# rasmusab/bayes.js

Hardware: AMD Instinct MI355X
Metric: posterior draws/sec (= param-updates/sec) (higher is better)
Workload: dtype f64

## Files before the change

### bayes.js_amd/csrc/amwg_kernel.h

```cpp
#pragma once
#if !defined(__HIPCC_RTC__)
#include <hip/hip_runtime.h>
#endif

#include "amwg_div.h"
#include "amwg_ld.h"
#include "amwg_philox.h"
#include "amwg_types.h"

namespace amwg {

struct LdsLayout {
  uint32_t data, state, pls, cnt, tot, cc, adapt, pl, idx, perm, total, stride, logpls, bc, xw;
};
__host__ __device__ inline LdsLayout lds_layout(size_t data_bytes, int P, int CPB, int max_top, int n_named, bool multi = false) {
  LdsLayout L;
  uint32_t o = 0;
  L.stride = (uint32_t)P | 1u;
  L.data = o;  o += (uint32_t)((data_bytes + 15) & ~(size_t)15);
  L.state = o; o += L.stride * CPB * 8;
  L.pls = o;   o += L.stride * CPB * 8;
  L.cnt = o;   o += L.stride * CPB * 8;
  L.tot = o;   o += (L.stride * CPB * 4 + 15) & ~15u;
  L.cc = o;    o += (uint32_t)P * sizeof(CompConst);
  L.adapt = o; o += ((uint32_t)P + 7) & ~7u;
  L.pl = o;    o += (uint32_t)n_named * 20u;
  o = (o + 15) & ~15u;
  L.idx = o;   o += (max_top > 1) ? (((uint32_t)max_top * CPB * (max_top > kByteTop ? 2u : 1u) + 15) & ~15u) : 0;
  L.perm = o;  o += (n_named > kPackedNamed) ? (((uint32_t)n_named * CPB * 2u + 15) & ~15u) : 0;
  L.logpls = o; o += multi ? L.stride * CPB * 8 : 0;
  L.bc = o;     o += multi ? ((L.stride * CPB * 4 + 15) & ~15u) : 0;
  L.xw = o;     o += multi ? 2u * 16u * 8u : 0;
  L.total = (o + 15) & ~15u;
  return L;
}

template <class Model, bool FAST, int G, int U = Model::kUnroll>
__device__ __forceinline__ double pass_over_data(const typename Model::Pass &ps, int n_obs, int sub, double acc) {
  const int n_full = n_obs / G, rem = n_obs % G;
  int k = 0;
  for (; k + U <= n_full; k += U) {
    double t[U];
#pragma unroll
    for (int u = 0; u < U; ++u) t[u] = Model::template term<FAST>(ps, (k + u) * G + sub);
#pragma unroll
    for (int u = 0; u < U; ++u) acc += t[u];
  }
  for (; k < n_full; ++k) acc += Model::template term<FAST>(ps, k * G + sub);
  if (sub < rem) acc += Model::template term<FAST>(ps, n_full * G + sub);
  return acc;
}

struct CrossWave {
  double *buf;
  int parity;
};

template <class...> using void_of = void;

template <class M, class = void> struct BinaryOf { static constexpr bool value = true; };
template <class M> struct BinaryOf<M, void_of<decltype(M::kHasBinary)>> { static constexpr bool value = M::kHasBinary; };

template <class M, class = void> struct TracksState { static constexpr bool value = false; };
template <class M> struct TracksState<M, void_of<decltype(M::kTracksState)>> { static constexpr bool value = M::kTracksState; };

// ... 170 lines not shown
  }
  __device__ __forceinline__ void set_block(const Philox4 &w) { u0 = u53(w.w0, w.w1); u1 = u53(w.w2, w.w3); }
  __device__ __forceinline__ void fill() { set_block(block(b0 + (uint64_t)lane_in_chain, c2, c3, k0, k1)); }
  __device__ __forceinline__ void init(uint64_t seed, uint64_t chain, uint64_t consumed, int tid) {
    k0 = (uint32_t)seed; k1 = (uint32_t)(seed >> 32);
    c2 = (uint32_t)chain; c3 = (uint32_t)(chain >> 32);
    lane_in_chain = tid & (L - 1);
    base_lane = (tid & 63) & ~(L - 1);
    b0 = consumed >> 1;
    pos = (uint32_t)(consumed & 1u);
    fill();
  }
  __device__ __forceinline__ uint64_t consumed() const { return 2 * b0 + (uint64_t)pos; }
  __device__ __forceinline__ double next() {
    if constexpr (L == 64) {
      uint32_t p = (uint32_t)__builtin_amdgcn_readfirstlane((int)pos);
      if (p >= 128u) { b0 += 64ull; p = 0u; fill(); }
      const double mine = (p & 1u) ? u1 : u0;
      const int src = (int)(p >> 1);
      const uint32_t hi = (uint32_t)__builtin_amdgcn_readlane((int)(f64_bits(mine) >> 32), src);
      const uint32_t lo = (uint32_t)__builtin_amdgcn_readlane((int)(uint32_t)f64_bits(mine), src);
      pos = p + 1u;
      return bits_f64(((uint64_t)hi << 32) | (uint64_t)lo);
    } else {
      if (pos >= 2u * (uint32_t)L) { b0 += (uint64_t)L; pos = 0u; fill(); }
      double mine = (pos & 1u) ? u1 : u0;
      if constexpr (L > 1) mine = __shfl(mine, base_lane + (int)(pos >> 1), 64);
      ++pos;
      return mine;
    }
  }
};

template <int G>
__device__ __forceinline__ bool chain_true(bool c) {
#if defined(__HIP_DEVICE_COMPILE__)
  if constexpr (G >= 64) return __ballot(c) != 0ull;
#endif
  return c;
}

__device__ inline __attribute__((noinline)) int certified_test_wide(double dA, double eta, double u) {
  const double lo = dA - eta, hi = dA + eta;
  if (hi < -746.0) return -1;
  if (lo >= 0.0) return 1;
  if (!(eta < 0x1p+9) || !(u > 0x1p-60)) return 0;
  if (exp_v8(lo) * (1.0 - 0x1p-50) > u) return 1;
  if (exp_v8(hi) * (1.0 + 0x1p-50) < u) return -1;
  return 0;
}
__device__ __forceinline__ int certified_test(double dA, double eta, double ex, double u) {
  if (eta < 0x1p-7) return (ex * (1.0 - eta) > u && (u > 0.0 || dA > -700.0)) ? 1 : (ex * (1.0 + eta) < u ? -1 : 0);
  return certified_test_wide(dA, eta, u);
}

template <class Rng>
__device__ __forceinline__ double rnorm_js(Rng &rng, double mean, double sd) {
  constexpr int GU = Rng::kLanesPerChain;
  double u, v, q;
  bool again;
  do {
    u = rng.next();
    v = 1.7156 * (rng.next() - 0.5);
    const double x = u - 0.449871;
    const double y = __builtin_fabs(v) + 0.386595;
    q = x * x + y * (0.19600 * y - 0.25472 * x);
    again = false;
    if (chain_true<GU>(q > 0.27597)) again = chain_true<GU>(q > 0.27846) || chain_true<GU>(v * v > -4 * log_v8_cold(u) * u * u);
  } while (again);
  return (v / u) * sd + mean;
}

struct IndexColumn {
  unsigned char *base;
  int CPB;
  bool wide;
  __device__ __forceinline__ int get(int t) const {
    return wide ? (int)reinterpret_cast<const uint16_t *>(base)[t * CPB] : (int)base[t * CPB];
  }
  __device__ __forceinline__ void set(int t, int v) const {
    if (wide) reinterpret_cast<uint16_t *>(base)[t * CPB] = (uint16_t)v; else base[t * CPB] = (uint8_t)v;
  }
};
__device__ __forceinline__ uint32_t perm_get(uint64_t perm, int i) { return (uint32_t)(perm >> (4 * i)) & 0xFu; }
__device__ __forceinline__ uint64_t perm_swap(uint64_t perm, int i, int j) {
  const uint64_t d = ((perm >> (4 * i)) ^ (perm >> (4 * j))) & 0xFull;
  return perm ^ (d << (4 * i)) ^ (d << (4 * j));
}

__device__ __forceinline__ double js_max2(double a, double b) {
  if (a != a || b != b) return __builtin_nan("");
  if (a == b) return (a == 0 && __builtin_signbit(a)) ? b : a;
  return a > b ? a : b;
}

template <class M, int G, bool GL, bool SW = false> struct RngOf { using type = CoopStream<G>; };
template <class M, int G> struct RngOf<M, G, true, false> { using type = typename M::Stream; };
template <class M, int G> struct RngOf<M, G, false, true> { using type = typename M::SweepStream; };
template <class M, class = void> struct DynamicLdsOf { static constexpr bool value = false; };
template <class M> struct DynamicLdsOf<M, void_of<decltype(M::kDynamicLds)>> { static constexpr bool value = M::kDynamicLds; };
template <class M, bool GL> struct DataBytesOf {
  static __device__ __forceinline__ size_t get(const DataRef &d, int lanes, int threads) {
    if constexpr (DynamicLdsOf<M>::value) return M::lds_bytes_of(d, lanes, threads);
    else return M::lds_bytes(d.n_obs, d.G, lanes);
  }
};
template <class M> struct DataBytesOf<M, true> { static __device__ __forceinline__ size_t get(const DataRef &d, int, int threads) { return M::gl_lds_bytes(d.pad, threads / 64); } };

#if defined(__HIP_DEVICE_COMPILE__)
typedef const StepArgs __attribute__((address_space(4))) *cold_args_ptr;
__device__ __forceinline__ cold_args_ptr cold_args() {
  cold_args_ptr p = (cold_args_ptr)__builtin_amdgcn_kernarg_segment_ptr();
  asm volatile("" : "+s"(p));
  return p;
}
#else
typedef const StepArgs *cold_args_ptr;
__device__ inline cold_args_ptr cold_args() { return nullptr; }
#endif

struct SlotPre {
  int comp;
  double cur, sd, batch_size;
  int2 cnt;
  bool adapting;
};

__device__ __forceinline__ uint64_t uniform_u64(uint64_t v) {
#if defined(__HIP_DEVICE_COMPILE__)
  return ((uint64_t)(uint32_t)__builtin_amdgcn_readfirstlane((int)(uint32_t)(v >> 32)) << 32) | (uint64_t)(uint32_t)__builtin_amdgcn_readfirstlane((int)(uint32_t)v);
// ... 68 lines not shown
}

__device__ __forceinline__ double lane_value(double v, int src) {
#if defined(__HIP_DEVICE_COMPILE__)
  const uint32_t hi = (uint32_t)__builtin_amdgcn_readlane((int)(f64_bits(v) >> 32), src);
  const uint32_t lo = (uint32_t)__builtin_amdgcn_readlane((int)(uint32_t)f64_bits(v), src);
  return bits_f64(((uint64_t)hi << 32) | (uint64_t)lo);
#else
  return v;
#endif
}

constexpr int kErrReplicasNeedOneWave = 1, kErrLaunchTooLong = 2, kErrMirrorOutOfSync = 4, kErrSweepNeedsOrderInRegisters = 8, kErrNoKernelBody = 16;
__device__ __forceinline__ void device_error(const StepArgs &a, int code) {
#if defined(__HIP_DEVICE_COMPILE__)
  if (threadIdx.x == 0) (void)atomicOr(a.ch.error, code);
#endif
}
template <class M, class = void> struct MirrorCheckOf { static constexpr bool value = false; };
template <class M> struct MirrorCheckOf<M, void_of<decltype(M::kMirrorCheck)>> { static constexpr bool value = M::kMirrorCheck; };

template <class Model, int G, int BT = 256, bool GL = false, bool SW = false, bool CT = false>
__device__ __forceinline__ void step_body(const StepArgs &a, unsigned char *smem) {
  constexpr int kPassU = SW ? (CertNeedsRows<Model>::value ? 2 : 4) : (BT >= 1024 ? 4 : 8);
  const int tid = threadIdx.x, nt = blockDim.x;
  constexpr bool kMulti = G > 64;
  if (!kMulti && a.cpb > 0 && nt != 64) { device_error(a, kErrReplicasNeedOneWave); return; }
  if (a.n_steps > 65535) { device_error(a, kErrLaunchTooLong); return; }
  const int CPB = kMulti ? G / 64 : ((a.cpb > 0 && a.cpb < nt / G) ? a.cpb : nt / G);
  const int c_raw = kMulti ? tid / 64 : tid / G;
  const int c_in = c_raw < CPB ? c_raw : CPB - 1, sub = tid % G;
  const int P = a.pl.P;
  const int n_named = a.pl.n_params;
  const LdsLayout L = lds_layout(DataBytesOf<Model, GL>::get(a.d, G, nt), P, CPB, a.pl.max_top, n_named, kMulti);

  const unsigned char *data_lds = smem + L.data;
  double *Sblk = reinterpret_cast<double *>(smem + L.state);
  CompConst *cc = reinterpret_cast<CompConst *>(smem + L.cc);
  uint8_t *adapt = smem + L.adapt;
  int32_t *pl_base = reinterpret_cast<int32_t *>(smem + L.pl), *pl_len = pl_base + n_named, *pl_top = pl_len + n_named, *pl_multidim = pl_top + n_named, *pl_inner = pl_multidim + n_named;
  const bool wide_idx = a.pl.max_top > kByteTop, wide_perm = n_named > kPackedNamed;
  const IndexColumn idx{smem + L.idx + (wide_idx ? 2 * c_in : c_in), CPB, wide_idx};
  const IndexColumn pcol{smem + L.perm + 2 * c_in, CPB, true};
  double *SDme = reinterpret_cast<double *>(smem + L.pls) + (size_t)c_in * L.stride;
  int2 *CNTme = reinterpret_cast<int2 *>(smem + L.cnt) + (size_t)c_in * L.stride;
  uint32_t *TOTme = reinterpret_cast<uint32_t *>(smem + L.tot) + (size_t)c_in * L.stride;
  double *LOGPLSme = reinterpret_cast<double *>(smem + L.logpls) + (size_t)c_in * L.stride;
  int32_t *BCme = reinterpret_cast<int32_t *>(smem + L.bc) + (size_t)c_in * L.stride;
  CrossWave xw{reinterpret_cast<double *>(smem + L.xw), 0};
  typename CacheOf<Model>::type cache = CacheOf<Model>::init();

  Model::stage(smem + L.data, a.d, tid, nt, G);
  for (int p = tid; p < P; p += nt) { cc[p] = a.cc[p]; adapt[p] = a.is_adapting[p]; }
  for (int i = tid; i < 4 * n_named; i += nt) pl_base[i] = a.pl.tab[i];
  for (int i = tid; i < n_named; i += nt) pl_inner[i] = a.pl.tab[n_named + i] / a.pl.tab[2 * n_named + i];

  const int64_t chain_raw = kMulti ? (int64_t)blockIdx.x : (int64_t)blockIdx.x * CPB + c_in;
  const bool live = chain_raw < a.C;
  const int64_t cl = live ? chain_raw : a.C - 1;
  const bool writer = live && sub == 0;
  const bool counter = sub == 0 && c_raw < CPB;
  const int64_t C = a.C;

  double *Sme = Sblk + (size_t)c_in * L.stride;
  for (int p = 0; p < P; ++p) {
    Sme[p] = a.ch.state[p * C + cl];
    SDme[p] = exp_v8(a.ch.prop_log_scale[p * C + cl]);
    CNTme[p] = make_int2(a.ch.acceptance_count[p * C + cl], a.ch.iterations_since_adaption[p * C + cl]);
    TOTme[p] = 0u;
    if constexpr (kMulti) { LOGPLSme[p] = a.ch.prop_log_scale[p * C + cl]; BCme[p] = a.ch.batch_count[p * C + cl]; }
  }
  const StateView S{Sme};
  uint64_t perm = wide_perm ? 0ull : a.ch.perm[cl];
  if (wide_perm)
    for (int k = 0; k < n_named; ++k) pcol.set(k, (int)a.ch.perm16[(int64_t)k * C + cl]);
  typename RngOf<Model, G, GL, SW>::type rng;
  if constexpr (GL) rng.init(a.seed, a.chain_offset + (uint64_t)cl, a.ch.rng_n[cl], tid, reinterpret_cast<double *>(smem + L.data + Model::gl_lds_bytes(a.d.pad, 0)) + (size_t)(tid >> 6) * 256);
  else if constexpr (SW) rng.init(a.seed, a.chain_offset + (uint64_t)cl, a.ch.rng_n[cl], tid, reinterpret_cast<double *>(smem + L.data + Model::window_offset(a.d, nt / 64)) + (size_t)(tid >> 6) * 256);
  else rng.init(a.seed, a.chain_offset + (uint64_t)cl, a.ch.rng_n[cl], tid);
  double lp_curr = a.ch.lp_curr[cl];
  __syncthreads();
  constexpr bool kCert = CT && CertifiedAt<Model, G>::value && !GL && (SW == CertNeedsRows<Model>::value);
  static_assert(kCert == CT, "a certified kernel is instantiated for a model that has no certified value at this lane count");
  constexpr bool kRefOrder = kCert && G > 1 && RefOrderOf<Model>::value;
  auto expression = [&]() -> double {
    if constexpr (kRefOrder) return Model::template reference_order<G>(cache, S, a.mc, a.d, data_lds, sub);
    else if constexpr (!GL) return log_post<Model, G, kPassU>(S, a, data_lds, sub, xw, cache);
    else return 0.0;
  };
  if constexpr (!GL) { if (a.init_lp) lp_curr = expression(); }
  double lpA = lp_curr, epsA = 0.0;
  bool lp_exact = true;
  if constexpr (kCert) { if (!a.init_lp) { epsA = a.ch.lp_eps[cl]; lp_exact = epsA == 0.0; } }
  (void)lpA; (void)epsA; (void)lp_exact;
#if defined(AMWG_AUDIT)
  constexpr bool kAudit = kCert;
#else
  constexpr bool kAudit = false;
#endif
  [[maybe_unused]] double audE = 0.0, aud_max_v = 0.0, aud_max_d = 0.0;
  [[maybe_unused]] uint32_t aud_n = 0u, aud_bad = 0u;
  [[maybe_unused]] auto audit_bin = [&](int which, double ratio) {
#if defined(AMWG_AUDIT)
    if (writer) {
      int b = 0;
      if (ratio > 0.0) { b = (int)((f64_bits(ratio) >> 52) & 0x7ffu) - 1023 + 40; b = b < 1 ? 1 : (b > 63 ? 63 : b); }
      if (!(ratio == ratio)) b = 63;
      (void)atomicAdd(cold_args()->ch.audit_hist + which * 64 + b, 1ull);
    }
#endif
  };
// ... 44 lines not shown

  const int lane64 = tid & 63;
  int ord = lane64;
  (void)ord;
  if (SW && a.pl.max_top > 64) { device_error(a, kErrSweepNeedsOrderInRegisters); return; }
  const bool ord_in_regs = SW ? true : (G >= 64 && a.pl.max_top <= 64);
  constexpr bool kSweep = SW && !GL && LaneReuseOf<Model>::value && G == 64 && !BinaryOf<Model>::value;
  const bool sweep_rt = kSweep && ord_in_regs && a.d.pad > 0;
  if constexpr (kAudit) { if (lp_exact) audE = lp_curr; else audE = expression(); }
  wave_priority(kStepperPriority);
  auto record_draws = [&](int step) {
    if (recording && step == next_rec) {
      double *const draws = cold_args()->draws;
      {
        constexpr int LW = G < 64 ? G : 64;
        if (live && (!kMulti || sub < 64))
          for (int p = sub & (LW - 1); p < P; p += LW) {
#if !defined(AMWG_X_NOREC)
            draws[(row * PR + p) * C + cl] = S(p);
#endif
          }
      }
      if constexpr (D > 0) {
        double dv[D];
        (void)Model::template eval<G, true>(S, a.d, data_lds, sub, dv);
        if (writer)
          for (int q = 0; q < D; ++q) draws[(row * PR + P + q) * C + cl] = dv[q];
      }
      ++row;
      next_rec += cold_args()->thin;
    }
  };
  auto shuffle_named = [&]() {
    for (int i = n_named - 1; i > 0; --i) {
      const int j = (int)__builtin_floor(rng.next() * (double)(i + 1));
      if (wide_perm) { const int ti = pcol.get(i); pcol.set(i, pcol.get(j)); pcol.set(j, ti); }
      else perm = perm_swap(perm, i, j);
    }
  };
  auto adapt_component = [&](int comp, bool accepted, int2 cnt, double batch_size, bool store, bool per_lane = false) {
    cnt.x += accepted ? 1 : 0;
    cnt.y += 1;
    const bool boundary = (double)cnt.y >= batch_size;
    if (per_lane ? boundary : chain_true<GL ? 1 : G>(boundary)) {
      const CompConst k = cc[comp];
      const int64_t gi = (int64_t)comp * C + cl;
      int32_t *const g_bc = kMulti ? nullptr : cold_args()->ch.batch_count;
      double *const g_pls = kMulti ? nullptr : cold_args()->ch.prop_log_scale;
      const int32_t bc = (kMulti ? BCme[comp] : g_bc[gi]) + 1;
      const double adj = __builtin_fmin(k.max_adaptation, k.initial_adaptation / __builtin_sqrt((double)bc));
      double pls = kMulti ? LOGPLSme[comp] : g_pls[gi];
      if ((double)cnt.x / k.batch_size > k.target_accept_rate) pls += adj; else pls -= adj;
      cnt = make_int2(0, 0);
      SDme[comp] = exp_v8_cold(pls);
      if constexpr (kMulti) { BCme[comp] = bc; LOGPLSme[comp] = pls; }
      else if (store) { g_bc[gi] = bc; g_pls[gi] = pls; }
    }
    CNTme[comp] = cnt;
  };

  [[maybe_unused]] auto accept_sweep = [&](double diff, double u_accept) -> bool {
    bool accepted = false;
    if (chain_true<G>(diff >= 0.0)) accepted = true;
    else if (chain_true<G>(diff < -746.0)) accepted = false;
    else {
      const double lower = 1.0 + diff;
// ... 532 lines not shown
        else {
          const double lower = 1.0 + diff;
          if (chain_true<G>(u_accept < lower - 0x1p-50)) accepted = true;
          else if (chain_true<G>(diff > -1.0 && u_accept > (lower + 0.5 * diff * diff) + 0x1p-50)) accepted = false;
          else accepted = chain_true<G>(exp_v8(diff) > u_accept);
        }
        accepted = chain_true<G>(accepted);
        if (accepted) lp_curr = prop_lp;
        else set_state(comp, cur);
        if constexpr (kCert) { lpA = lp_curr; epsA = 0.0; }
        if (counter) (void)__hip_atomic_fetch_add(&TOTme[comp], 1u + (accepted ? 0x10000u : 0u), __ATOMIC_RELAXED, __HIP_MEMORY_SCOPE_WORKGROUP);
      }
      if constexpr (kAudit) { if (inb && accepted) audE = aud_E_prop; }
      AMWG_PHASE(11);
      if (chain_true<G>(me.adapting)) adapt_component(comp, accepted, me.cnt, me.batch_size, writer);
      AMWG_PHASE(12);
    }
  }

  if constexpr (kCert) {
    if (a.finalize_lp && !lp_exact) { lp_curr = expression(); lp_exact = true; }
    if (!lp_exact) lp_curr = lpA;
    if (writer) cold_args()->ch.lp_eps[cl] = lp_exact ? 0.0 : epsA;
  }
  if constexpr (!GL && MirrorCheckOf<Model>::value) {
    if (!Model::template mirror_ok<G>(cache, S, a.d, sub)) (void)atomicOr(cold_args()->ch.error, kErrMirrorOutOfSync);
  }
#if defined(AMWG_X_PHASES)
  if ((tid & 63) == 0 && live) {
    unsigned long long *const hh = cold_args()->ch.audit_hist + 64;
#pragma unroll
    for (int q = 0; q < 16; ++q) (void)atomicAdd(hh + q, (unsigned long long)ph_acc[q]);
  }
#endif
  if constexpr (kAudit) {
    if (writer) {
      double *const au = cold_args()->ch.audit;
      const double v0 = au[cl], d0 = au[C + cl];
      au[cl] = (aud_max_v > v0 || !(aud_max_v == aud_max_v)) ? aud_max_v : v0;
      au[C + cl] = (aud_max_d > d0 || !(aud_max_d == aud_max_d)) ? aud_max_d : d0;
      au[2 * C + cl] += (double)aud_n;
      au[3 * C + cl] += (double)aud_bad;
    }
  }
  if (writer) {
    const cold_args_ptr ca = cold_args();
    double *const o_state = ca->ch.state, *const o_pls = ca->ch.prop_log_scale;
    int32_t *const o_ac = ca->ch.acceptance_count, *const o_it = ca->ch.iterations_since_adaption, *const o_bc = ca->ch.batch_count;
    int32_t *const o_acc = ca->ch.accepts, *const o_inb = ca->ch.inbounds;
    for (int p = 0; p < P; ++p) {
      o_state[p * C + cl] = S(p);
      o_ac[p * C + cl] = CNTme[p].x;
      o_it[p * C + cl] = CNTme[p].y;
      o_acc[p * C + cl] += (int32_t)(TOTme[p] >> 16);
      o_inb[p * C + cl] += (int32_t)(TOTme[p] & 0xffffu);
      if constexpr (kMulti) { o_pls[p * C + cl] = LOGPLSme[p]; o_bc[p * C + cl] = BCme[p]; }
    }
    if (wide_perm) { uint16_t *const o_p16 = ca->ch.perm16; for (int k = 0; k < n_named; ++k) o_p16[(int64_t)k * C + cl] = (uint16_t)pcol.get(k); }
    else ca->ch.perm[cl] = perm;
    ca->ch.rng_n[cl] = rng.consumed();
    ca->ch.lp_curr[cl] = lp_curr;
  }
}

template <class M, class = void> struct MinWavesOf { static constexpr int value = 1; };
template <class M> struct MinWavesOf<M, void_of<decltype(M::kMinWavesPerSimd)>> { static constexpr int value = M::kMinWavesPerSimd; };
// ... 29 lines not shown
```

### bayes.js_amd/csrc/amwg_plan.hip

```cpp
#include <algorithm>
#include <cmath>
#include <cstdlib>

#include "amwg_host.h"
#include "amwg_kernel.h"
#include "amwg_models.h"

using namespace amwg;

const FamilyRow *family_of(int model) {
  static const FamilyRow rows[4] = {amwg_family_row<0>(), amwg_family_row<1>(), amwg_family_row<2>(), amwg_family_row<3>()};
  return model >= AMWG_MODEL_NORMAL && model <= AMWG_MODEL_POIS_GLM ? &rows[model - 1] : nullptr;
}

int gl_layout(const double *y, const int32_t *g, int N, int Gn, GlLayoutHost *out) {
  if (Gn < 1 || Gn > 64) return amwg_fail(AMWG_EINVAL, "group_local: 1 to 64 groups (a chain runs on one wavefront, a lane serves one group), got %d", Gn);
  std::vector<int> n(Gn, 0), L(Gn, 1), first(Gn, 0);
  for (int i = 0; i < N; ++i) {
    if (g[i] < 0 || g[i] >= Gn) return amwg_fail(AMWG_EINVAL, "group_local: g[%d] = %d outside 0..%d", i, g[i], Gn - 1);
    n[g[i]]++;
  }
  int total = Gn;
  for (;;) {
    int best = 0;
// ... 59 lines not shown
    p.pad = rows ? HierNormalModel::row_pitch(s->user_rows_n) : 0;
    if (rows && s->user_rows_sweep && !s->user_has_binary && s->pl.max_top <= 64)
      p.variant = cert && s->user_rows_cert ? Variant::UserSweepCert : Variant::UserSweep;
    else
      p.variant = cert && ((s->user_cert_tail_n > 0 && G == 1) || ((s->user_pois_tail_n > 0 || s->user_logit_tail_n > 0) && G == 16)) ? Variant::UserStepCert : Variant::UserStep;
    return p;
  }
  if (s->mc.group_local) { p.variant = Variant::GroupLocal, p.pad = s->gl_rounds; return p; }
  const bool rows = s->model == AMWG_MODEL_HIER_NORMAL && rows_wanted && ((s->hier_periodic_mask >> 6) & 1u) && s->d.G <= 64 && s->d.n_obs >= 64 &&
                    rows_fit(HierNormalModel::row_pitch(s->d.n_obs), s->d.G);
  const bool cert = decide_certified && ((s->model == AMWG_MODEL_NORMAL && G == 1) || (s->model == AMWG_MODEL_POIS_GLM && G == 16) || rows) &&
                    family_of(s->model)->certified(G, bt) != nullptr;
  p.variant = rows ? (cert ? Variant::HierSweepCert : Variant::HierSweep) : (cert ? Variant::StepCert : Variant::Step);
  p.pad = rows ? HierNormalModel::row_pitch(s->d.n_obs) : ((cert && s->model == AMWG_MODEL_NORMAL && bt <= 512 && !o.sufficient_statistics) ? 1 : 0);
  return p;
}

static bool row_layout(const amwg_sampler *s, const LaunchPlan &p) {
  return p.variant == Variant::HierSweep || p.variant == Variant::HierSweepCert || (s->user && p.pad > 0);
}

static uint32_t lds_of(const amwg_sampler *s, const LaunchPlan &p, int cpb = 0) {
  const int G = p.lanes, bt = p.block;
  size_t data = 0;
  switch (p.variant) {
    case Variant::GroupLocal: data = HierGlModel::gl_lds_bytes(p.pad, bt / 64); break;
    case Variant::HierSweep: case Variant::HierSweepCert: data = HierNormalModel::rows_lds_bytes(p.pad, bt / 64, s->d.G); break;
    case Variant::Step: case Variant::StepCert:
      data = (s->model == AMWG_MODEL_NORMAL && G == 1) ? (p.pad ? NormalModel::one_lane_tile_bytes(s->d.n_obs) : 0) : family_of(s->model)->lds_bytes(s->d.n_obs, s->d.G, G);
      break;
    default:
      data = p.pad ? HierNormalModel::rows_lds_bytes(p.pad, bt / 64, s->user_rows_groups) : (size_t)(G == 1 ? s->user_lds_one_lane : s->user_lds);
  }
  return G > 64 ? lds_layout(data, s->P, G / 64, s->pl.max_top, s->n_params, true).total : lds_layout(data, s->P, cpb ? cpb : bt / G, s->pl.max_top, s->n_params).total;
}

static int log2_of(int lanes) { int lg = 0; for (int g = lanes; g > 1; g >>= 1) ++lg; return lg; }
static double model_work(const amwg_sampler *s, int G) {
  const LaunchPlan q = variant_for(s, G, 256, (size_t)160 * 1024);
  const double N = (double)s->d.n_obs;
  switch (s->model) {
    case AMWG_MODEL_NORMAL: return q.variant == Variant::StepCert ? (s->opt.sufficient_statistics ? 40.0 : 2.6 * N) : 9.0 * N;
    case AMWG_MODEL_BETA_BERN:
      return G == 1 ? (s->mc.exact_division ? 1.8 * N : 400.0 * (1.0 + std::log2(N + 2.0))) : 6.0 * N;
    case AMWG_MODEL_HIER_NORMAL: {
      const bool periodic = ((s->hier_periodic_mask >> log2_of(G)) & 1u) != 0;
      double w = (periodic ? 8.6 : 12.0) * N + 12.0 * s->d.G;
      if (row_layout(s, q)) w *= (2.0 + 0.35 * s->d.G) / (2.0 + s->d.G);
      return w;
    }
    case AMWG_MODEL_POIS_GLM: return q.variant == Variant::StepCert ? 36.0 * N : 90.0 * N;
  }
  if (q.variant == Variant::UserStepCert && s->user_pois_tail_n > 0) {
    const double n = (double)s->user_pois_tail_n, w = s->user_work > 0 ? s->user_work : 1e6;
    return (w - 70.0 * n > 0.4 * w) ? w - 70.0 * n : 0.4 * w;
  }
  if (q.variant == Variant::UserStepCert && s->user_logit_tail_n > 0) {
    return 0.36 * (s->user_work > 0 ? s->user_work : 1e6);
  }
  if (q.variant == Variant::UserStepCert) {
    const double w1 = s->user_work_one_lane > 0 ? s->user_work_one_lane : s->user_work, n = (double)s->user_cert_tail_n;
    return (w1 - 16.0 * n > 0 ? w1 - 16.0 * n : 0.0) + 2.6 * n;
  }
  if (G == 1 && s->user_work_one_lane > 0) return s->user_work_one_lane;
  double w = s->user_work > 0 ? s->user_work : 1e6;
  if (row_layout(s, q)) w *= (2.0 + 0.35 * s->user_rows_groups) / (2.0 + s->user_rows_groups);
  return w;
// ... 34 lines not shown
    return amwg_fail(AMWG_EINVAL, "this closure has no loop that can be split over lanes: lanes_per_chain must be 1 (or 0 = auto), got %d", lanes);
  const int bts[5] = {1024, 512, 256, 128, 64};
  LaunchPlan best, one;
  double best_cost = -1.0, cost1 = -1.0;
  const bool fixed_lanes = lanes > 0;
  for (int G = 1; G <= 1024; G <<= 1) {
    if (fixed_lanes && G != lanes) continue;
    if (s->user && !s->user_parallel && G > 1) break;
    if (s->user && s->user_parallel && !fixed_lanes && G == 1 && !(s->user_work_one_lane > 0) && variant_for(s, 1, 256, max_lds).variant != Variant::UserStepCert) continue;
    int pick = 0;
    for (int bi = 0; bi < 5; ++bi) {
      const int bt = bts[bi];
      if (o.block_threads && bt != o.block_threads) continue;
      if (G > 64 && bt != G) continue;
      if (!fits(bt, G)) continue;
      pick = bt;
      if ((s->C + bt / G - 1) / (bt / G) >= n_cus) break;
    }
    int cpb = 0;
    if (!pick && G < 64 && max_bt >= 64 && (!o.block_threads || o.block_threads == 64)) {
      for (int c = 32 / G; c >= 1; c >>= 1)
        if (lds_of(s, variant_for(s, G, 64, max_lds), c) <= max_lds) { pick = 64; cpb = c; break; }
    }
    if (!pick) continue;
    LaunchPlan p = variant_for(s, G, pick, max_lds);
    p.cpb = cpb;
    const int CPB = cpb ? cpb : pick / G;
    const int64_t blocks = (s->C + CPB - 1) / CPB;
    const uint32_t lds = lds_of(s, p, cpb);
    int64_t per_cu = 2048 / pick;
    if (lds > 0 && (int64_t)(max_lds / lds) < per_cu) per_cu = (int64_t)(max_lds / lds);
    if (per_cu < 1) per_cu = 1;
    const int64_t resident = blocks < per_cu * n_cus ? blocks : per_cu * n_cus;
    const double w_res = (double)resident * (pick / 64) / (4.0 * n_cus);
    const double w_total = (double)blocks * (pick / 64) / (4.0 * n_cus);
    const double S = 400.0 + 97.0 * (G < 64 ? 6 - log2_of(G) : 0);
    const double Wl = model_work(s, G) / G + (G > 64 ? 150.0 : 0.0);
    const double w1 = w_res > 1.0 ? w_res : 1.0;
    const double cost = (w_total / w_res) * (S * (w_res > 1.8 ? w_res : 1.8) + Wl * w1 * (1.0 + 0.14 / w1));
    if (G == 1) { cost1 = cost; one = p; }
    if (best_cost < 0 || cost < best_cost * (1.0 - 1e-9)) { best_cost = cost; best = p; }
  }
  if (lanes == 0 && best.lanes > 1 && cost1 > 0 && cost1 <= 1.12 * best_cost) best = one;
  if (!best.lanes) return amwg_fail(AMWG_EINVAL, "no launch geometry fits: the model needs more than %zu bytes of LDS", max_lds);
  const int CPB = best.lanes > 64 ? 1 : (best.cpb ? best.cpb : best.block / best.lanes);
  best.grid = (int)((s->C + CPB - 1) / CPB);
  best.lds = (int)lds_of(s, best, best.cpb);
  *out = best;
  return AMWG_OK;
}

int adopt_plan(amwg_sampler *s, const LaunchPlan &p) {
  s->plan = p;
  s->d.pad = p.pad;
  if (s->user) return size_wave_scratch(s);
  if (s->model == AMWG_MODEL_HIER_NORMAL) s->mc.group_lane_const = (int32_t)((s->hier_periodic_mask >> log2_of(p.lanes)) & 1u);
  switch (p.variant) {
    case Variant::StepCert: case Variant::HierSweepCert: s->kernel = family_of(s->model)->certified(p.lanes, p.block); break;
    case Variant::HierSweep: s->kernel = amwg_kernel_hier_sweep(p.block); break;
    case Variant::GroupLocal: s->kernel = amwg_kernel_hier_gl(p.block); break;
    default: s->kernel = family_of(s->model)->kernel(p.lanes, p.block);
  }
  if (!s->kernel) return amwg_fail(AMWG_EINVAL, "no kernel for model %d with %d lanes per chain in workgroups of %d", s->model, p.lanes, p.block);
  return size_wave_scratch(s);
}
struct TuneCandidate { LaunchPlan plan; hipModule_t module; hipFunction_t fn; float ms; };
// ... 67 lines not shown
```

### bayes.js_amd/csrc/amwg_run.hip

```cpp
#include <dlfcn.h>
#include <sys/mman.h>

#include <cmath>
#include <cstdlib>

#include "../../include/amwg_selftest.h"
#include "amwg_host.h"
#include "amwg_kernel.h"

using namespace amwg;

int use_device(int device) {
  int ndev = 0;
  hipError_t e = hipGetDeviceCount(&ndev);
  if (e != hipSuccess || ndev < 1) return amwg_fail(AMWG_EHIP, "no HIP device available (%s)", hipGetErrorString(e));
  HIP_TRY(hipSetDevice(device));
  return AMWG_OK;
}

namespace {
struct Roctx {
  int (*push)(const char *) = nullptr;
  int (*pop)() = nullptr;
  Roctx() {
// ... 6 lines not shown
      pop = reinterpret_cast<int (*)()>(dlsym(h, "roctxRangePop"));
      if (!push || !pop) push = nullptr, pop = nullptr;
    }
  }
};
Roctx &roctx() { static Roctx r; return r; }
}

int launch_steps(amwg_sampler *s, int64_t n, int64_t thin, double *d_draws, bool finalize) {
  Roctx &rx = roctx();
  if (rx.push) rx.push(d_draws ? "amwg_sample" : "amwg_burn");
  struct PopOnExit { Roctx &r; ~PopOnExit() { if (r.pop) r.pop(); } } pop_on_exit{rx};
  int64_t chunk = (s->opt.steps_per_launch > 0 && s->opt.steps_per_launch < 65535) ? s->opt.steps_per_launch : 65535;
  if (d_draws && d_draws == s->d_draws && s->opt.steps_per_launch <= 0) {
    const double per_step = (double)(s->P + s->D) * (double)s->C * 8.0 / (double)thin;
    const double steps = 33554432.0 / (per_step > 0 ? per_step : 1.0);
    if (steps < (double)chunk) chunk = steps < 16.0 ? 16 : (int64_t)steps;
  }
  const LaunchPlan &p = s->plan;
  if (p.cpb > 0 && p.block != 64) return amwg_fail(AMWG_EINVAL, "internal: %d chains per workgroup of %d threads (replicated chains need one-wavefront workgroups)", p.cpb, p.block);
  if (p.lanes == 1 && s->d.wave_scratch && wave_scratch_lines(s) < (size_t)p.grid * (size_t)(p.block / 64))
    return amwg_fail(AMWG_EINVAL, "internal: a wave scratch of %zu lines for %d workgroups of %d threads (one line per wavefront)", wave_scratch_lines(s), p.grid, p.block);
  if (chunk > 65535) return amwg_fail(AMWG_EINVAL, "internal: launches of %lld steps (at most 65535)", (long long)chunk);
  StepArgs a{};
  a.C = s->C;
  a.seed = s->opt.seed;
  a.chain_offset = s->opt.chain_offset;
  a.thin = (int32_t)thin;
  a.draws = d_draws;
  a.cc = s->d_cc;
  a.is_adapting = s->d_adapt;
  a.pl = s->pl;
  a.cpb = p.cpb;
  a.sweep_update_by_update = s->opt.full_evaluation == 2 ? 1 : 0;
  a.certified = info(p.variant).certified ? 1 : 0;
  a.bound_scale = std::ldexp(1.0, s->opt.test_bound_shift);
  a.audit_adversarial = 0;
#if defined(AMWG_AUDIT)
  { const char *e = getenv("AMWG_AUDIT_ADVERSARIAL"); a.audit_adversarial = (e && e[0] == '1') ? 1 : 0; }
#endif
  a.mc = s->mc;
  a.d = s->d;
  if (p.lanes != 1) a.d.wave_scratch = nullptr;
  a.ch = s->ch;
  const bool quiet = finalize && n == 0 && s->lp_ready;
  if (!quiet) {
    s->n_launches = 0;
    s->chunk_rows.clear();
    HIP_TRY(hipEventRecord(s->ev0, s->stream));
  }
  int64_t done = 0, row = 0;
  do {
    const int64_t m = (n - done < chunk) ? n - done : chunk;
    a.n_steps = (int32_t)m;
    a.init_lp = s->lp_ready ? 0 : 1;
    a.finalize_lp = finalize ? 1 : 0;
    a.step0 = (thin - (done % thin)) % thin;
    a.row0 = row;
    if (s->user) {
      size_t arg_bytes = sizeof a;
      void *extra[] = {HIP_LAUNCH_PARAM_BUFFER_POINTER, &a, HIP_LAUNCH_PARAM_BUFFER_SIZE, &arg_bytes, HIP_LAUNCH_PARAM_END};
      HIP_TRY(hipModuleLaunchKernel(s->user_fn, (unsigned)p.grid, 1, 1, (unsigned)p.block, 1, 1, (unsigned)p.lds, s->stream, nullptr, extra));
    } else {
      hipLaunchKernelGGL(s->kernel, dim3(p.grid), dim3(p.block), (size_t)p.lds, s->stream, a);
      HIP_TRY(hipGetLastError());
    }
// ... 258 lines not shown
```

### bayes.js_amd/csrc/amwg_sampler.h

```cpp
#pragma once
#include <hip/hip_runtime.h>

#include <cstdint>
#include <string>
#include <utility>
#include <vector>

#include "../../include/amwg.h"
#include "amwg_types.h"

typedef void (*step_kernel_t)(const amwg::StepArgs);

enum class Variant : uint8_t {
  Step, StepCert, HierSweep, HierSweepCert, GroupLocal,
  UserStep, UserStepCert, UserSweep, UserSweepCert
};
struct LaunchPlan {
  int lanes = 0, block = 0, grid = 0, lds = 0, cpb = 0;
  Variant variant = Variant::Step;
  int pad = 0;
};

struct amwg_sampler {
  int device = 0;
  hipStream_t stream = nullptr;
  hipEvent_t ev0 = nullptr, ev1 = nullptr;
  int model = 0, P = 0, n_params = 0;
  int64_t C = 0;
  amwg_options opt{};
  amwg::ParamLayout pl{};
  amwg::ModelConsts mc{};
  amwg::DataRef d{};
  amwg::ChainArrays ch{};
  std::vector<void *> dev_allocs;
  amwg::CompConst *d_cc = nullptr;
  uint8_t *d_adapt = nullptr;
  std::vector<uint8_t> h_adapt;
  std::vector<int32_t> h_layout;
  LaunchPlan plan;
  step_kernel_t kernel = nullptr;
  int gl_rounds = 0;
  std::string kernel_name;
  uint32_t hier_periodic_mask = 0;
  bool lp_ready = false;
  bool lp_is_expression = true;
  std::vector<std::pair<int, float>> tuned;
  bool user = false;
  int D = 0;
  int user_lds = 0, user_lds_one_lane = 0, user_parallel = 0, user_max_threads = 1024;
  int user_rows_n = 0, user_rows_groups = 0, user_rows_sweep = 0;
  bool user_rows_cert = false;
// ... 21 lines not shown
```

### bayes.js_amd/csrc/amwg_types.h

```cpp
#pragma once
#include "amwg_stdint.h"

namespace amwg {

constexpr int kPackedNamed = 16;
constexpr int kByteTop = 256;
constexpr int kMaxIndex = 65535;
constexpr int kInlineUserArrays = 16;
constexpr int kTypeReal = 0, kTypeInt = 1, kTypeBinary = 2, kTypeFixed = 3;

struct StateView {
  const double *base;
#if defined(__HIPCC__)
  __host__ __device__ __forceinline__
#else
  inline
#endif
  double operator()(int p) const { return base[p]; }
};

struct CompConst {
  double lower, upper, max_adaptation, initial_adaptation, target_accept_rate;
  double batch_size;
  int32_t type;
// ... 36 lines not shown
};

struct ChainArrays {
  double *state;
  double *prop_log_scale;
  int32_t *acceptance_count, *iterations_since_adaption, *batch_count;
  int32_t *accepts, *inbounds;
  uint64_t *perm;
  uint16_t *perm16;
  uint64_t *rng_n;
  double *lp_curr;
  double *lp_eps;
  double *audit;
  unsigned long long *audit_hist;
  int32_t *error;
};

struct StepArgs {
  int64_t C;
  uint64_t seed, chain_offset;
  int32_t n_steps, thin;
  int64_t step0;
  double *draws;
  int64_t row0;
  const CompConst *cc;
  const uint8_t *is_adapting;
  int32_t init_lp;
  int32_t finalize_lp;
  int32_t certified;
  double bound_scale;
  int32_t audit_adversarial;
  int32_t sweep_update_by_update;
  int32_t cpb;
  ParamLayout pl;
  ModelConsts mc;
  DataRef d;
  ChainArrays ch;
};

}
```

Before: 1.403 billion.

## Add LDS-backed Philox ring buffer stream for one-lane-per-chain kernels

Adds a RingStream RNG for the G==1 step path. It pre-generates Philox uniforms into a per-thread ring in LDS, filled in wave-uniform rounds before each proposal's normal draw and before the named-parameter shuffle, so lanes that need extra draws from rejection sampling no longer diverge on Philox generation. The planner picks a ring size (16 down to 2 slots) that fits the LDS budget for the chosen occupancy. This costs extra LDS traffic, some extra Philox blocks generated ahead of use, and possibly LDS pressure.

```diff
diff --git a/bayes.js_amd/csrc/amwg_kernel.h b/bayes.js_amd/csrc/amwg_kernel.h
--- a/bayes.js_amd/csrc/amwg_kernel.h
+++ b/bayes.js_amd/csrc/amwg_kernel.h
@@ -11,9 +11,9 @@
 namespace amwg {
 
 struct LdsLayout {
-  uint32_t data, state, pls, cnt, tot, cc, adapt, pl, idx, perm, total, stride, logpls, bc, xw;
+  uint32_t data, state, pls, cnt, tot, cc, adapt, pl, idx, perm, total, stride, logpls, bc, xw, ring;
 };
-__host__ __device__ inline LdsLayout lds_layout(size_t data_bytes, int P, int CPB, int max_top, int n_named, bool multi = false) {
+__host__ __device__ inline LdsLayout lds_layout(size_t data_bytes, int P, int CPB, int max_top, int n_named, bool multi = false, size_t ring_bytes = 0) {
   LdsLayout L;
   uint32_t o = 0;
   L.stride = (uint32_t)P | 1u;
@@ -31,6 +31,9 @@
   L.logpls = o; o += multi ? L.stride * CPB * 8 : 0;
   L.bc = o;     o += multi ? ((L.stride * CPB * 4 + 15) & ~15u) : 0;
   L.xw = o;     o += multi ? 2u * 16u * 8u : 0;
+  o = (o + 15) & ~15u;
+  if (ring_bytes > 0 && max_top <= 1) o += ((uint32_t)CPB + 15) & ~15u;
+  L.ring = o;   o += (uint32_t)ring_bytes;
   L.total = (o + 15) & ~15u;
   return L;
 }
@@ -267,6 +270,97 @@
   }
 };
 
+__device__ __forceinline__ uint32_t lds_byte_offset(const unsigned char *p) {
+#if defined(__HIP_DEVICE_COMPILE__)
+  return (uint32_t)(uintptr_t)(__attribute__((address_space(3))) const unsigned char *)p;
+#else
+  return 0u;
+#endif
+}
+
+struct RingStream {
+  static constexpr int kLanesPerChain = 1;
+  static constexpr uint32_t kUpdateNeed = 6u;
+  uint32_t k0, k1, c2, c3;
+  uint64_t b_base;
+  uint32_t pos, end;
+  uint32_t K, sh;
+  uint32_t ring;
+#if defined(AMWG_X_PHASES)
+  uint32_t ev[3];
+  __device__ __forceinline__ void count(int i, uint32_t n = 1u) { if ((int)(threadIdx.x & 63u) == __ffsll((unsigned long long)__ballot(1)) - 1) ev[i] += n; }
+#else
+  __device__ __forceinline__ void count(int, uint32_t = 1u) {}
+#endif
+#if defined(__HIP_DEVICE_COMPILE__)
+  typedef __attribute__((address_space(3))) double *LdsDouble;
+  __device__ __forceinline__ LdsDouble slot(uint32_t at) const { return (LdsDouble)(uintptr_t)(ring + ((at & (K - 1u)) << sh)); }
+#else
+  __device__ __forceinline__ double *slot(uint32_t) const { return nullptr; }
+#endif
+  static __device__ __attribute__((noinline)) Philox4 block(uint64_t b, uint32_t c2, uint32_t c3, uint32_t k0, uint32_t k1) {
+    return philox4x32_10((uint32_t)b, (uint32_t)(b >> 32), c2, c3, k0, k1);
+  }
+  __device__ __forceinline__ void init(uint64_t seed, uint64_t chain, uint64_t consumed, uint32_t ring_offset, int slots, int threads) {
+    k0 = (uint32_t)seed; k1 = (uint32_t)(seed >> 32);
+    c2 = (uint32_t)chain; c3 = (uint32_t)(chain >> 32);
+    b_base = consumed >> 1;
+    pos = (uint32_t)(consumed & 1u);
+    end = 0u;
+    K = (uint32_t)slots;
+    sh = 3u + (uint32_t)(31 - __builtin_clz((unsigned)threads));
+    ring = ring_offset;
+#if defined(AMWG_X_PHASES)
+    ev[0] = ev[1] = ev[2] = 0u;
+#endif
+  }
+  __device__ __forceinline__ uint64_t consumed() const { return 2 * b_base + (uint64_t)pos; }
+  __device__ __forceinline__ int held() const { return (int)(end - pos); }
+  static __device__ __attribute__((noinline)) uint32_t fill_rounds(uint32_t k0, uint32_t k1, uint32_t c2, uint32_t c3, uint64_t b_base, uint32_t pos, uint32_t end,
+                                                                    uint32_t K, uint32_t sh, uint32_t ring, int need, bool active) {
+#if defined(__HIP_DEVICE_COMPILE__)
+    do {
+      if ((int)(end - pos) + 2 <= (int)K) {
+        const uint64_t b = b_base + (uint64_t)(end >> 1);
+        const Philox4 w = philox4x32_10((uint32_t)b, (uint32_t)(b >> 32), c2, c3, k0, k1);
+        const LdsDouble p = (LdsDouble)(uintptr_t)(ring + ((end & (K - 1u)) << sh));
+        p[0] = u53(w.w0, w.w1);
+        *(LdsDouble)(uintptr_t)(ring + (((end + 1u) & (K - 1u)) << sh)) = u53(w.w2, w.w3);
+        end += 2u;
+      }
+    } while (__ballot(active && (int)(end - pos) < need) != 0ull);
+#endif
+    return end;
+  }
+  __device__ __forceinline__ void top_up(uint32_t need, bool active = true) {
+#if defined(__HIP_DEVICE_COMPILE__)
+    if (K == 0u) return;
+    const int n = (int)(need < K ? need : K - 1u);
+    if (__ballot(active && held() < n) != 0ull) {
+      [[maybe_unused]] const uint32_t end0 = end;
+      end = fill_rounds(k0, k1, c2, c3, b_base, pos, end, K, sh, ring, n, active);
+#if defined(AMWG_X_PHASES)
+      uint32_t rounds = 0u;
+      while (__ballot(((end - end0) >> 1) > rounds) != 0ull) ++rounds;
+      count(0, rounds);
+#endif
+    }
+#endif
+  }
+  __device__ __forceinline__ double next() {
+    if (held() <= 0) {
+      count(0);
+      if (K == 0u) {
+        const uint64_t b = b_base + (uint64_t)(pos >> 1);
+        const Philox4 w = block(b, c2, c3, k0, k1);
+        return (pos++ & 1u) ? u53(w.w2, w.w3) : u53(w.w0, w.w1);
+      }
+      end = fill_rounds(k0, k1, c2, c3, b_base, pos, pos & ~1u, K, sh, ring, 0, false);
+    }
+    return *slot(pos++);
+  }
+};
+
 template <int G>
 __device__ __forceinline__ bool chain_true(bool c) {
 #if defined(__HIP_DEVICE_COMPILE__)
@@ -305,6 +399,31 @@
   } while (again);
   return (v / u) * sd + mean;
 }
+__device__ __forceinline__ double rnorm_js(RingStream &rng, double mean, double sd) {
+  double u = 1.0, v = 0.0;
+  [[maybe_unused]] bool again = true;
+#if defined(__HIP_DEVICE_COMPILE__)
+  uint32_t need = RingStream::kUpdateNeed;
+  do {
+    rng.top_up(need, again);
+    need = 3u;
+    rng.count(1);
+    if (again) {
+      u = rng.next();
+      v = 1.7156 * (rng.next() - 0.5);
+      const double x = u - 0.449871;
+      const double y = __builtin_fabs(v) + 0.386595;
+      const double q = x * x + y * (0.19600 * y - 0.25472 * x);
+      again = false;
+      if (q > 0.27597) {
+        again = q > 0.27846;
+        if (!again) { rng.count(2); again = v * v > -4 * log_v8_cold(u) * u * u; }
+      }
+    }
+  } while (__ballot(again) != 0ull);
+#endif
+  return (v / u) * sd + mean;
+}
 
 struct IndexColumn {
   unsigned char *base;
@@ -331,6 +450,7 @@
 
 template <class M, int G, bool GL, bool SW = false> struct RngOf { using type = CoopStream<G>; };
 template <class M, int G> struct RngOf<M, G, true, false> { using type = typename M::Stream; };
+template <class M> struct RngOf<M, 1, false, false> { using type = RingStream; };
 template <class M, int G> struct RngOf<M, G, false, true> { using type = typename M::SweepStream; };
 template <class M, class = void> struct DynamicLdsOf { static constexpr bool value = false; };
 template <class M> struct DynamicLdsOf<M, void_of<decltype(M::kDynamicLds)>> { static constexpr bool value = M::kDynamicLds; };
@@ -465,7 +585,8 @@
   const int c_in = c_raw < CPB ? c_raw : CPB - 1, sub = tid % G;
   const int P = a.pl.P;
   const int n_named = a.pl.n_params;
-  const LdsLayout L = lds_layout(DataBytesOf<Model, GL>::get(a.d, G, nt), P, CPB, a.pl.max_top, n_named, kMulti);
+  constexpr bool kRing = G == 1 && !GL && !SW;
+  const LdsLayout L = lds_layout(DataBytesOf<Model, GL>::get(a.d, G, nt), P, CPB, a.pl.max_top, n_named, kMulti, kRing ? (size_t)a.rng_ring * (size_t)nt * 8 : 0);
 
   const unsigned char *data_lds = smem + L.data;
   double *Sblk = reinterpret_cast<double *>(smem + L.state);
@@ -510,6 +631,7 @@
   typename RngOf<Model, G, GL, SW>::type rng;
   if constexpr (GL) rng.init(a.seed, a.chain_offset + (uint64_t)cl, a.ch.rng_n[cl], tid, reinterpret_cast<double *>(smem + L.data + Model::gl_lds_bytes(a.d.pad, 0)) + (size_t)(tid >> 6) * 256);
   else if constexpr (SW) rng.init(a.seed, a.chain_offset + (uint64_t)cl, a.ch.rng_n[cl], tid, reinterpret_cast<double *>(smem + L.data + Model::window_offset(a.d, nt / 64)) + (size_t)(tid >> 6) * 256);
+  else if constexpr (kRing) rng.init(a.seed, a.chain_offset + (uint64_t)cl, a.ch.rng_n[cl], lds_byte_offset(smem + L.ring) + 8u * (uint32_t)tid, a.rng_ring, nt);
   else rng.init(a.seed, a.chain_offset + (uint64_t)cl, a.ch.rng_n[cl], tid);
   double lp_curr = a.ch.lp_curr[cl];
   __syncthreads();
@@ -620,6 +742,7 @@
     }
   };
   auto shuffle_named = [&]() {
+    if constexpr (kRing) rng.top_up((uint32_t)(n_named - 1));
     for (int i = n_named - 1; i > 0; --i) {
       const int j = (int)__builtin_floor(rng.next() * (double)(i + 1));
       if (wide_perm) { const int ti = pcol.get(i); pcol.set(i, pcol.get(j)); pcol.set(j, ti); }
@@ -1218,6 +1341,9 @@
 #pragma unroll
     for (int q = 0; q < 16; ++q) (void)atomicAdd(hh + q, (unsigned long long)ph_acc[q]);
   }
+  if constexpr (kRing) {
+    for (int q = 0; q < 3; ++q) if (rng.ev[q] != 0u) (void)atomicAdd(cold_args()->ch.audit_hist + 80 + q, (unsigned long long)rng.ev[q]);
+  }
 #endif
   if constexpr (kAudit) {
     if (writer) {
diff --git a/bayes.js_amd/csrc/amwg_plan.hip b/bayes.js_amd/csrc/amwg_plan.hip
--- a/bayes.js_amd/csrc/amwg_plan.hip
+++ b/bayes.js_amd/csrc/amwg_plan.hip
@@ -115,7 +115,15 @@
     default:
       data = p.pad ? HierNormalModel::rows_lds_bytes(p.pad, bt / 64, s->user_rows_groups) : (size_t)(G == 1 ? s->user_lds_one_lane : s->user_lds);
   }
-  return G > 64 ? lds_layout(data, s->P, G / 64, s->pl.max_top, s->n_params, true).total : lds_layout(data, s->P, cpb ? cpb : bt / G, s->pl.max_top, s->n_params).total;
+  const size_t ring = G == 1 ? (size_t)p.ring * (size_t)bt * 8 : 0;
+  return G > 64 ? lds_layout(data, s->P, G / 64, s->pl.max_top, s->n_params, true).total : lds_layout(data, s->P, cpb ? cpb : bt / G, s->pl.max_top, s->n_params, false, ring).total;
+}
+
+static int ring_slots(const amwg_sampler *s, LaunchPlan p, int64_t per_cu, size_t max_lds) {
+  const size_t budget = max_lds / (size_t)(per_cu > 0 ? per_cu : 1);
+  for (p.ring = 16; p.ring >= 2; p.ring >>= 1)
+    if ((size_t)lds_of(s, p, p.cpb) <= budget) return p.ring;
+  return 0;
 }
 
 static int log2_of(int lanes) { int lg = 0; for (int g = lanes; g > 1; g >>= 1) ++lg; return lg; }
@@ -216,6 +224,7 @@
     if (lds > 0 && (int64_t)(max_lds / lds) < per_cu) per_cu = (int64_t)(max_lds / lds);
     if (per_cu < 1) per_cu = 1;
     const int64_t resident = blocks < per_cu * n_cus ? blocks : per_cu * n_cus;
+    if (G == 1) p.ring = ring_slots(s, p, (resident + n_cus - 1) / n_cus, max_lds);
     const double w_res = (double)resident * (pick / 64) / (4.0 * n_cus);
     const double w_total = (double)blocks * (pick / 64) / (4.0 * n_cus);
     const double S = 400.0 + 97.0 * (G < 64 ? 6 - log2_of(G) : 0);
diff --git a/bayes.js_amd/csrc/amwg_run.hip b/bayes.js_amd/csrc/amwg_run.hip
--- a/bayes.js_amd/csrc/amwg_run.hip
+++ b/bayes.js_amd/csrc/amwg_run.hip
@@ -62,6 +62,7 @@
   a.is_adapting = s->d_adapt;
   a.pl = s->pl;
   a.cpb = p.cpb;
+  a.rng_ring = p.ring;
   a.sweep_update_by_update = s->opt.full_evaluation == 2 ? 1 : 0;
   a.certified = info(p.variant).certified ? 1 : 0;
   a.bound_scale = std::ldexp(1.0, s->opt.test_bound_shift);
diff --git a/bayes.js_amd/csrc/amwg_sampler.h b/bayes.js_amd/csrc/amwg_sampler.h
--- a/bayes.js_amd/csrc/amwg_sampler.h
+++ b/bayes.js_amd/csrc/amwg_sampler.h
@@ -16,7 +16,7 @@
   UserStep, UserStepCert, UserSweep, UserSweepCert
 };
 struct LaunchPlan {
-  int lanes = 0, block = 0, grid = 0, lds = 0, cpb = 0;
+  int lanes = 0, block = 0, grid = 0, lds = 0, cpb = 0, ring = 0;
   Variant variant = Variant::Step;
   int pad = 0;
 };
diff --git a/bayes.js_amd/csrc/amwg_types.h b/bayes.js_amd/csrc/amwg_types.h
--- a/bayes.js_amd/csrc/amwg_types.h
+++ b/bayes.js_amd/csrc/amwg_types.h
@@ -92,6 +92,7 @@
   int32_t audit_adversarial;
   int32_t sweep_update_by_update;
   int32_t cpb;
+  int32_t rng_ring;
   ParamLayout pl;
   ModelConsts mc;
   DataRef d;
```

Measured after the change: 1.402 billion. About the same (-0.1%).
